# tobias-kirschstein/nersemble

Measured on NVIDIA H100. Metric: M ray-samples/sec, higher is better.
Workload: dtype f16 tables/MLP operands, f32 accumulate

## Files before the change

### nersemble_b200/csrc/nsb_field.cu

```cuda
#include <algorithm>
#include <cstdlib>
#include <cstring>

#define NSB_NO_SPIN_GUARD 1
#include "nsb_common.cuh"
#include "nsb_gather.cuh"
#include "nsb_march.cuh"
#include "nsb_mlp.cuh"
#include "nsb_tc.cuh"

namespace nsb {

constexpr int kSlabBytes = 2048;
constexpr int kChunkSlabs = 4;
constexpr int kChunkBytes = kSlabBytes * kChunkSlabs;
constexpr int kStages = 4;
constexpr int kBiasFloats = 6 * 128 + 8;

struct FieldArgs {
    nsb_field_params P;
    nsb_field_opts O;
    nsb_samples S;
    nsb_field_out out;
    float aabb_size[3];
// ... 198 lines not shown
        ha[0][1] = pack_h2(g02, b1acc[0][3]);
        ha[0][2] = pack_h2(b1acc[1][0], b1acc[1][1]);
        ha[0][3] = pack_h2(b1acc[1][2], b1acc[1][3]);
        float e[2][2];
#pragma unroll
        for (int h = 0; h < 2; ++h) {
            const int r = g + 8 * h;
            const float d0 = (dirsel[r][0] + 1.0f) / 2.0f, d1 = (dirsel[r][1] + 1.0f) / 2.0f,
                        d2 = (dirsel[r][2] + 1.0f) / 2.0f;
            e[h][0] = q == 0 ? d0 : (q == 1 ? d2 : 1.0f);
            e[h][1] = q == 0 ? d1 : 1.0f;
        }
        ha[1][0] = pack_h2(e[0][0], e[0][1]);
        ha[1][1] = pack_h2(e[1][0], e[1][1]);
        ha[1][2] = pack_h2(1.0f, 1.0f);
        ha[1][3] = pack_h2(1.0f, 1.0f);
    }
    float c0acc[8][4];
    smem_gemm<2, 4>(c0acc, ha, field_w + 384, lane);
    uint32_t c1in[4][4];
    relu_pack_nobias<8>(c0acc, c1in);
    float c1acc[8][4];
    smem_gemm<4, 4>(c1acc, c1in, field_w + 640, lane);
    uint32_t c2in[4][4];
    relu_pack_nobias<8>(c1acc, c2in);
    float c2acc[2][4];
    smem_gemm<4, 1>(c2acc, c2in, field_w + 1152, lane);
    if (A.out.rgb) {
        const int64_t sa = row0 + g, sb = row0 + g + 8;
        if (q == 0) {
            if (sa < n) { A.out.rgb[3 * sa + 0] = 1.f / (1.f + expf(-c2acc[0][0])); A.out.rgb[3 * sa + 1] = 1.f / (1.f + expf(-c2acc[0][1])); }
            if (sb < n) { A.out.rgb[3 * sb + 0] = 1.f / (1.f + expf(-c2acc[0][2])); A.out.rgb[3 * sb + 1] = 1.f / (1.f + expf(-c2acc[0][3])); }
        } else if (q == 1) {
            if (sa < n) A.out.rgb[3 * sa + 2] = 1.f / (1.f + expf(-c2acc[0][0]));
            if (sb < n) A.out.rgb[3 * sb + 2] = 1.f / (1.f + expf(-c2acc[0][2]));
        }
    }
}

template <bool DEFORM, bool FIELD, bool HEAD, bool SAVE>
__global__ void __launch_bounds__(kLaunchBoundWS, 1) field_kernel_ws(const __grid_constant__ FieldArgs A) {
    extern __shared__ __align__(1024) uint8_t smem_raw[];
    SmemWS &sm = *reinterpret_cast<SmemWS *>(smem_raw);
    const int tid = threadIdx.x, lane = tid & 31, warp = tid >> 5;
    constexpr bool FEAT_GIVEN = false;

#define NSB_N_SAMPLES A.S.n_samples
#include "nsb_field_setup.inc"
    if (warp >= kTensorWarps) {
        if (kGatherRegs != kLaunchRegs) asm volatile("setmaxnreg.dec.sync.aligned.u32 %0;" ::"n"(kGatherRegs));
#include "nsb_field_gather_role.inc"
        return;
    }

    if (kTensorRegs != kLaunchRegs) asm volatile("setmaxnreg.inc.sync.aligned.u32 %0;" ::"n"(kTensorRegs));
#include "nsb_field_tensor_role.inc"
#undef NSB_N_SAMPLES
}

template <bool DEFORM>
__global__ void __launch_bounds__(kLaunchBoundWS, 1) field_kernel_ws_given(const __grid_constant__ FieldArgs A) {
    extern __shared__ __align__(1024) uint8_t smem_raw[];
    SmemWS &sm = *reinterpret_cast<SmemWS *>(smem_raw);
    const int tid = threadIdx.x, lane = tid & 31, warp = tid >> 5;
    constexpr bool FIELD = true, HEAD = true, SAVE = true, FEAT_GIVEN = true;
#define NSB_N_SAMPLES A.S.n_samples
#include "nsb_field_setup.inc"
    if (warp >= kTensorWarps) {
        if (kGatherRegs != kLaunchRegs) asm volatile("setmaxnreg.dec.sync.aligned.u32 %0;" ::"n"(kGatherRegs));
#include "nsb_field_gather_role.inc"
        return;
    }
    if (kTensorRegs != kLaunchRegs) asm volatile("setmaxnreg.inc.sync.aligned.u32 %0;" ::"n"(kTensorRegs));
#include "nsb_field_tensor_role.inc"
#undef NSB_N_SAMPLES
}

#ifndef NSB_FRAME_GATHER_WARPS
#define NSB_FRAME_GATHER_WARPS 8
#endif
constexpr int kFrameGatherWarps = NSB_FRAME_GATHER_WARPS;
constexpr int kTcStages = 4, kTcBlocksPerTile = 14;
#ifdef NSB_TC_PROF
constexpr int kTcProfPhases = 9;
__device__ unsigned long long g_tc_prof[kTcProfPhases], g_tc_prof_k[8];
#define KPROF(i) if (threadIdx.x == 0 && blockIdx.x == 3) g_tc_prof_k[i] = (unsigned long long)clock64();
#else
#define KPROF(i)
#endif
constexpr size_t kTcPackedBytes = 12 * 16384 + 2 * 2048;

__device__ __forceinline__ int tc_warp_index(int tid) { return __shfl_sync(0xffffffffu, tid >> 5, 0); }

struct alignas(1024) SmemTC {
    uint8_t wring[kTcStages][16384];
    uint8_t a_enc[16384];
    uint4 field_w[kFieldPackedU4];
    alignas(16) float bias[kBiasFloats];
    alignas(16) float heads[2][64][8];
    uint64_t full[kTcStages];
    uint64_t xs_full[2], feat_full[2];
    uint32_t ring_rel[kTcStages];
    int row_ts[NSB_TILE];
    int tile_ctr[2];
    int64_t n_dyn;
    uint64_t sampler_done;
    alignas(16) float xs[2][NSB_TILE][4];
    alignas(16) __half feat[2][NSB_TILE * kFeatStride];
    alignas(16) float dirsel[2][NSB_TILE][4];
    uint2 blend_b[kGatherWarps][4 * 32];
    uint4 cv_stage[kGatherWarps][1];
};
static_assert(sizeof(SmemTC) <= 227 * 1024, "shared memory plan");
static_assert(kTensorWarps == 8, "the wgmma tensor role runs two warpgroups of 64 rows");

#define NSB_TC_SETUP()                                                                                              \
    {                                                                                                               \
        const uint4 *src = reinterpret_cast<const uint4 *>(A.P.field_packed);                                      \
        for (int i = tid; i < kFieldPackedU4; i += kThreadsWS) sm.field_w[i] = __ldg(src + i);                     \
        for (int i = tid; i < kBiasFloats; i += kThreadsWS) sm.bias[i] = __ldg(A.P.deform_bias + i);               \
        for (int i = tid; i < (int)(sizeof(sm.a_enc) / 16); i += kThreadsWS) reinterpret_cast<uint4 *>(&sm.a_enc)[i] = make_uint4(0u, 0u, 0u, 0u); \
        if (tid == 0) {                                                                                             \
            for (int s = 0; s < kTcStages; ++s) { mbar_init(&sm.full[s], 1); sm.ring_rel[s] = 0; }                \
            for (int b = 0; b < 2; ++b) {                                                                           \
                mbar_init(&sm.xs_full[b], kTensorWarps);                                                            \
                mbar_init(&sm.feat_full[b], kGatherWarps);                                                          \
                sm.tile_ctr[b] = 0;                                                                                 \
            }                                                                                                       \
            mbar_fence_init();                                                                                      \
        }                                                                                                           \
        __syncthreads();                                                                                            \
    }

template <bool HEAD, bool FRAME, bool STACK>
__global__ void __launch_bounds__(kLaunchBoundWS, 1) field_kernel_tc(const __grid_constant__ FieldArgs A) {
    extern __shared__ __align__(1024) uint8_t smem_raw[];
    SmemTC &sm = *reinterpret_cast<SmemTC *>(smem_raw);
    const int tid = threadIdx.x, lane = tid & 31, warp = tc_warp_index(tid);
    constexpr bool FIELD = true, SAVE = false, FEAT_GIVEN = false;
#define NSB_N_SAMPLES A.S.n_samples
    NSB_TC_SETUP()
    if (warp >= kTensorWarps) {
        if (kGatherRegs != kLaunchRegs) asm volatile("setmaxnreg.dec.sync.aligned.u32 %0;" ::"n"(kGatherRegs));
        if constexpr (FRAME) {
#include "nsb_field_gather_role_frame.inc"
        } else {
#include "nsb_field_gather_role.inc"
        }
        return;
    }
    if (kTensorRegs != kLaunchRegs) asm volatile("setmaxnreg.inc.sync.aligned.u32 %0;" ::"n"(kTensorRegs));
#include "nsb_field_tensor_role_tc.inc"
#undef NSB_N_SAMPLES
}

template <bool DEFORM, bool FIELD, bool HEAD, bool SAVE>
__global__ void __launch_bounds__(kLaunchBoundWS, 1) field_kernel_ws_dyn(const __grid_constant__ FieldArgs A) {
    extern __shared__ __align__(1024) uint8_t smem_raw[];
    SmemWS &sm = *reinterpret_cast<SmemWS *>(smem_raw);
    const int tid = threadIdx.x, lane = tid & 31, warp = tid >> 5;
    constexpr bool FEAT_GIVEN = false;
    if (tid == 0) sm.n_dyn = min(*A.S.n_samples_dev, A.S.n_samples);
#define NSB_N_SAMPLES (*reinterpret_cast<const volatile int64_t *>(&sm.n_dyn))
#include "nsb_field_setup.inc"
    if (warp >= kTensorWarps) {
        if (kGatherRegs != kLaunchRegs) asm volatile("setmaxnreg.dec.sync.aligned.u32 %0;" ::"n"(kGatherRegs));
#include "nsb_field_gather_role.inc"
        return;
    }
    if (kTensorRegs != kLaunchRegs) asm volatile("setmaxnreg.inc.sync.aligned.u32 %0;" ::"n"(kTensorRegs));
#include "nsb_field_tensor_role.inc"
#undef NSB_N_SAMPLES
}

struct RenderKArgs {
    FieldArgs F;
    nsb_march_args M;
    nsb_composite_args C;
    int32_t sampler, n_per_ray;
    float near_plane;
    int64_t capacity;
    nsb_render_ws_header *hdr;
    int64_t *partials;
    int64_t *packed_info;
};

__device__ __forceinline__ uint32_t ld_acquire_u32(const uint32_t *p) {
    uint32_t v;
    asm volatile("ld.acquire.gpu.global.u32 %0, [%1];" : "=r"(v) : "l"(p) : "memory");
    return v;
}
__device__ __forceinline__ void phase_sync() { asm volatile("bar.sync 1, %0;" ::"n"(kTensorWarps * 32) : "memory"); }
__device__ __forceinline__ void grid_barrier(uint32_t *ctr, const uint32_t target) {
    phase_sync();
    if (threadIdx.x == 0) {
        __threadfence();
        atomicAdd(ctr, 1u);
        while (ld_acquire_u32(ctr) < target) __nanosleep(40);
        __threadfence();
    }
    phase_sync();
}

__device__ __forceinline__ int64_t phase_sum_i64(int64_t v, int64_t *smem_warp , const int tid) {
// ... 208 lines not shown
    nsb_field_params P;
    nsb_field_opts O;
    const float *x;
    const float *codes;
    int64_t n;
    void *out;
    int out_is_half;
};

__global__ void __launch_bounds__(256) hash_blend_kernel(const __grid_constant__ HashArgs H) {
    const int lane = threadIdx.x & 31;
    const int64_t warp_global = (int64_t)blockIdx.x * (blockDim.x >> 5) + (threadIdx.x >> 5);
    const int64_t n_warps = (int64_t)gridDim.x * (blockDim.x >> 5);
    for (int64_t s = warp_global; s < H.n; s += n_warps) {
        const float x = H.x[3 * s + 0], y = H.x[3 * s + 1], z = H.x[3 * s + 2];
#if NSB_GATHER_MMA
        const BlendB Bf = make_blend_b(H.O, H.codes + s * NSB_MEMBERS, lane);
        const float val = gather_blend_mma(H.P, x, y, z, Bf, lane);
#else
        const int mg = lane & 7;
        float4 c = __ldg(reinterpret_cast<const float4 *>(H.codes + s * NSB_MEMBERS) + mg);
        float cw[4];
        cw[0] = fmaf(c.x, H.O.cw_scale[4 * mg + 0], H.O.cw_bias[4 * mg + 0]);
        cw[1] = fmaf(c.y, H.O.cw_scale[4 * mg + 1], H.O.cw_bias[4 * mg + 1]);
        cw[2] = fmaf(c.z, H.O.cw_scale[4 * mg + 2], H.O.cw_bias[4 * mg + 2]);
        cw[3] = fmaf(c.w, H.O.cw_scale[4 * mg + 3], H.O.cw_bias[4 * mg + 3]);
        const float val = gather_blend<2>(H.P, x, y, z, cw, lane);
#endif
        if (H.out_is_half)
            reinterpret_cast<__half *>(H.out)[s * 32 + lane] = __float2half_rn(val);
        else
            reinterpret_cast<float *>(H.out)[s * 32 + lane] = val;
    }
}

static int g_num_sms = 0;
static int num_sms() {
    if (g_num_sms == 0) {
        int dev = 0;
        cudaGetDevice(&dev);
        cudaDeviceGetAttribute(&g_num_sms, cudaDevAttrMultiProcessorCount, dev);
        if (g_num_sms <= 0) g_num_sms = 132;
    }
    return g_num_sms;
}

template <bool D, bool F, bool H, bool SV>
static int launch_field_ws_(const FieldArgs &A, cudaStream_t st) {
    const size_t smem = sizeof(SmemWS);
    static bool configured = false;
    if (!configured) {
        cudaError_t e = cudaFuncSetAttribute(field_kernel_ws<D, F, H, SV>, cudaFuncAttributeMaxDynamicSharedMemorySize, (int)smem);
        if (e != cudaSuccess) {
            set_error("cudaFuncSetAttribute(field_kernel_ws): %s", cudaGetErrorString(e));
            return 1;
        }
        configured = true;
    }
    const int64_t n_tiles = (A.S.n_samples + NSB_TILE - 1) / NSB_TILE;
    const int grid = (int)std::min<int64_t>(n_tiles, (int64_t)num_sms());
    field_kernel_ws<D, F, H, SV><<<grid, kThreadsWS, smem, st>>>(A);
    return check_launch("field_kernel_ws");
}
template <bool D, bool F, bool H, bool SV>
static int launch_field_ws_dyn_(const FieldArgs &A, cudaStream_t st) {
    const size_t smem = sizeof(SmemWS);
    static bool configured = false;
    if (!configured) {
        cudaError_t e = cudaFuncSetAttribute(field_kernel_ws_dyn<D, F, H, SV>, cudaFuncAttributeMaxDynamicSharedMemorySize, (int)smem);
        if (e != cudaSuccess) { set_error("cudaFuncSetAttribute(field_kernel_ws_dyn): %s", cudaGetErrorString(e)); return 1; }
        configured = true;
    }
    const int64_t n_tiles = (A.S.n_samples + NSB_TILE - 1) / NSB_TILE;
    const int grid = (int)std::min<int64_t>(n_tiles, (int64_t)num_sms());
    field_kernel_ws_dyn<D, F, H, SV><<<grid, kThreadsWS, smem, st>>>(A);
    return check_launch("field_kernel_ws_dyn");
}
template <bool D, bool F, bool H>
static int launch_field_ws(const FieldArgs &A, cudaStream_t st) {
    const bool save = A.out.xs || A.out.deform_acts || A.out.deform_enc || A.out.corner_vals;
    return save ? launch_field_ws_<D, F, H, true>(A, st) : launch_field_ws_<D, F, H, false>(A, st);
}

template <bool H, bool FR, bool ST>
static int launch_field_tc_(const FieldArgs &A, cudaStream_t st) {
    const size_t smem = sizeof(SmemTC);
    static bool configured = false;
    if (!configured) {
        cudaError_t e = cudaFuncSetAttribute(field_kernel_tc<H, FR, ST>, cudaFuncAttributeMaxDynamicSharedMemorySize, (int)smem);
        if (e != cudaSuccess) { set_error("cudaFuncSetAttribute(field_kernel_tc): %s", cudaGetErrorString(e)); return 1; }
        configured = true;
    }
    const int64_t n_tiles = (A.S.n_samples + NSB_TILE - 1) / NSB_TILE;
    const int grid = (int)std::min<int64_t>(n_tiles, (int64_t)num_sms());
    field_kernel_tc<H, FR, ST><<<grid, kThreadsWS, smem, st>>>(A);
    return check_launch("field_kernel_tc");
}
template <bool H>
static int launch_field_tc(const FieldArgs &A, cudaStream_t st) {
    if (!A.P.frame_table) return launch_field_tc_<H, false, false>(A, st);
    return A.P.frame_stride ? launch_field_tc_<H, true, true>(A, st) : launch_field_tc_<H, true, false>(A, st);
}

template <bool D>
static int launch_field_given(const FieldArgs &A, cudaStream_t st) {
    const size_t smem = sizeof(SmemWS);
    static bool configured = false;
    if (!configured) {
        cudaError_t e = cudaFuncSetAttribute(field_kernel_ws_given<D>, cudaFuncAttributeMaxDynamicSharedMemorySize, (int)smem);
        if (e != cudaSuccess) { set_error("cudaFuncSetAttribute(field_kernel_ws_given): %s", cudaGetErrorString(e)); return 1; }
        configured = true;
    }
    const int64_t n_tiles = (A.S.n_samples + NSB_TILE - 1) / NSB_TILE;
    const int grid = (int)std::min<int64_t>(n_tiles, (int64_t)num_sms());
    field_kernel_ws_given<D><<<grid, kThreadsWS, smem, st>>>(A);
    return check_launch("field_kernel_ws_given");
}

static bool frame_stride_ok(const nsb_field_params *p) {
    return p->frame_stride >= 0 && p->frame_stride * (int64_t)p->n_timesteps <= (int64_t)UINT32_MAX;
}

template <bool D, bool F, bool H>
static int launch_field(const FieldArgs &A, cudaStream_t st) {
    if (A.S.given_feat) {
        if (F && H && !A.S.n_samples_dev) return launch_field_given<D>(A, st);
        set_error("nsb_field_forward: given_feat needs the full evaluation (rgb) and a host-side sample count");
        return 1;
    }
    if (A.S.n_samples_dev) {
        if (F && !H) return launch_field_ws_dyn_<D, true, false, true>(A, st);
        set_error("nsb_field_forward: n_samples_dev is supported for the density evaluation (no rgb) only");
        return 1;
    }
    if (D && F && A.P.deform_packed_umma && !A.S.sample_code_bias && !(A.out.xs || A.out.deform_acts || A.out.deform_enc || A.out.corner_vals || A.out.feat))
        return launch_field_tc<H>(A, st);
    return launch_field_ws<D, F, H>(A, st);
}

}

using namespace nsb;

extern "C" size_t nsb_deform_packed_bytes(void) { return (size_t)kTbNumSlabs * kSlabBytes; }
extern "C" size_t nsb_field_packed_bytes(void) { return kFieldPackedU4 * sizeof(uint4); }
extern "C" size_t nsb_deform_packed_umma_bytes(void) { return kTcPackedBytes; }
#ifdef NSB_TC_PROF
extern "C" int nsb_debug_tc_prof(unsigned long long *out) {
    return (int)cudaMemcpyFromSymbol(out, nsb::g_tc_prof, sizeof(unsigned long long) * kTcProfPhases);
}
extern "C" int nsb_debug_tc_prof_kernel(unsigned long long *out8) {
    return (int)cudaMemcpyFromSymbol(out8, nsb::g_tc_prof_k, sizeof(unsigned long long) * 8);
}
#endif

extern "C" int nsb_field_forward(const nsb_field_params *params, const nsb_field_opts *opts, const nsb_samples *samples,
                                 const nsb_field_out *out, void *stream) {
    if (!params || !opts || !samples || !out) { set_error("nsb_field_forward: null argument"); return 1; }
    if (samples->n_samples <= 0) return 0;
    if (params->levels.n_levels != NSB_MAX_LEVELS) { set_error("nsb_field_forward: n_levels must be 16"); return 1; }
    if (!samples->origins && !samples->positions) { set_error("nsb_field_forward: no sample source"); return 1; }
    if (samples->origins && (!samples->directions || !samples->t_starts || !samples->t_ends || !samples->ray_indices)) {
        set_error("nsb_field_forward: ray-based samples need directions, t_starts, t_ends, ray_indices");
        return 1;
    }
    const bool deform = opts->use_deformation != 0;
    const bool need_field = out->sigma || out->rgb || out->feat || out->xs;
    const bool head = opts->compute_rgb != 0 && out->rgb != nullptr;
    if (!need_field && !(deform && out->offsets)) { set_error("nsb_field_forward: no outputs requested"); return 1; }
    if (need_field && (!params->tables || !params->field_packed)) { set_error("nsb_field_forward: tables/field_packed missing"); return 1; }
    if (need_field && !params->blend_codes && !samples->sample_blend_codes) { set_error("nsb_field_forward: no blend codes"); return 1; }
    if (deform && (!params->deform_packed_tb || !params->deform_bias || (!params->deform_code_bias && !samples->sample_code_bias))) {
// ... 8 lines not shown
    if (!frame_stride_ok(params)) { set_error("nsb_field_forward: frame_stride out of range"); return 1; }
    FieldArgs A;
    A.P = *params; A.O = *opts; A.S = *samples; A.out = *out;
    for (int k = 0; k < 3; ++k) A.aabb_size[k] = params->aabb[3 + k] - params->aabb[k];
    cudaStream_t st = (cudaStream_t)stream;
    if (deform) {
        if (!need_field) return launch_field<true, false, false>(A, st);
        return head ? launch_field<true, true, true>(A, st) : launch_field<true, true, false>(A, st);
    }
    return head ? launch_field<false, true, true>(A, st) : launch_field<false, true, false>(A, st);
}

extern "C" int nsb_hash_blend_forward(const nsb_field_params *params, const nsb_field_opts *opts, const float *x,
                                      const float *codes, int64_t n, void *out, int32_t out_is_half, void *stream) {
    if (!params || !opts || !x || !codes || !out) { set_error("nsb_hash_blend_forward: null argument"); return 1; }
    if (n <= 0) return 0;
    if (params->levels.n_levels != NSB_MAX_LEVELS) { set_error("nsb_hash_blend_forward: n_levels must be 16"); return 1; }
    HashArgs H;
    H.P = *params; H.O = *opts; H.x = x; H.codes = codes; H.n = n; H.out = out; H.out_is_half = out_is_half;
    const int64_t warps_needed = n;
    const int blocks = (int)std::min<int64_t>((warps_needed + 7) / 8, (int64_t)num_sms() * 8);
    hash_blend_kernel<<<blocks, 256, 0, (cudaStream_t)stream>>>(H);
    return check_launch("hash_blend_kernel");
}

namespace nsb {
constexpr int kBlendMaxTimesteps = 256;
__global__ void __launch_bounds__(256) blend_tables_kernel(const uint4 *__restrict__ tables, const float *__restrict__ code,
                                                           const __grid_constant__ nsb_field_opts O, float2 *__restrict__ out,
                                                           int n_ts, int64_t n_entries) {
    __shared__ float4 cw_s[kBlendMaxTimesteps][8];
    const int lane = threadIdx.x & 31, sub = lane & 7;
    for (int i = threadIdx.x; i < n_ts * 8; i += blockDim.x) {
        const int t = i >> 3, s = i & 7;
        float cw[4];
#pragma unroll
        for (int k = 0; k < 4; ++k) cw[k] = fmaf(__ldg(code + t * NSB_MEMBERS + 4 * s + k), O.cw_scale[4 * s + k], O.cw_bias[4 * s + k]);
        cw_s[t][s] = make_float4(cw[0], cw[1], cw[2], cw[3]);
    }
    __syncthreads();
    const int64_t stride = (int64_t)gridDim.x * (blockDim.x >> 3);
    for (int64_t e = (int64_t)blockIdx.x * (blockDim.x >> 3) + (threadIdx.x >> 3); e < ((n_entries + 3) & ~(int64_t)3); e += stride) {
        float2 f[4] = {};
        if (e < n_entries) {
            const uint4 v = __ldcs(tables + e * 8 + sub);
            f[0] = unpack_h2(v.x); f[1] = unpack_h2(v.y); f[2] = unpack_h2(v.z); f[3] = unpack_h2(v.w);
        }
        for (int t = 0; t < n_ts; ++t) {
            const float4 c4 = cw_s[t][sub];
            const float cw[4] = {c4.x, c4.y, c4.z, c4.w};
            float f0 = 0.f, f1 = 0.f;
#pragma unroll
            for (int i = 0; i < 4; ++i) { f0 = fmaf(cw[i], f[i].x, f0); f1 = fmaf(cw[i], f[i].y, f1); }
#pragma unroll
            for (int o = 1; o < 8; o <<= 1) { f0 += __shfl_xor_sync(0xffffffffu, f0, o); f1 += __shfl_xor_sync(0xffffffffu, f1, o); }
            if (sub == 0 && e < n_entries) out[(int64_t)t * n_entries + e] = make_float2(f0, f1);
        }
    }
}
}

extern "C" int nsb_blend_tables(const nsb_field_params *params, const nsb_field_opts *opts, int32_t first_timestep,
                                int32_t n_timesteps, int64_t n_entries, void *out, void *stream) {
    if (!params || !opts || !out || !params->tables || !params->blend_codes) { set_error("nsb_blend_tables: null argument"); return 1; }
    if (first_timestep < 0 || n_timesteps < 1 || n_timesteps > kBlendMaxTimesteps || first_timestep > params->n_timesteps - n_timesteps) {
        set_error("nsb_blend_tables: timesteps [%d, %d + %d) out of range (n_timesteps %d, at most %d per call)", first_timestep,
                  first_timestep, n_timesteps, params->n_timesteps, kBlendMaxTimesteps);
        return 1;
    }
    if (n_entries <= 0) return 0;
    const int blocks = (int)std::min<int64_t>((n_entries + 31) / 32, (int64_t)num_sms() * 8);
    blend_tables_kernel<<<blocks, 256, 0, (cudaStream_t)stream>>>(reinterpret_cast<const uint4 *>(params->tables),
                                                                  params->blend_codes + (size_t)first_timestep * NSB_MEMBERS, *opts,
                                                                  reinterpret_cast<float2 *>(out), n_timesteps, n_entries);
    return check_launch("blend_tables_kernel");
}

namespace nsb {
constexpr size_t kRenderHdrBytes = 64, kRenderPartials = 1024;
static_assert(sizeof(nsb_render_ws_header) == kRenderHdrBytes, "workspace header layout");

template <int SAMPLER, bool FR, bool ST>
static int launch_render_tc_(const RenderKArgs &K, cudaStream_t st) {
    const size_t smem = sizeof(SmemTC);
    static bool configured = false;
    if (!configured) {
        cudaError_t e = cudaFuncSetAttribute(render_kernel_tc<SAMPLER, FR, ST>, cudaFuncAttributeMaxDynamicSharedMemorySize, (int)smem);
        if (e != cudaSuccess) { set_error("cudaFuncSetAttribute(render_kernel_tc): %s", cudaGetErrorString(e)); return 1; }
        configured = true;
    }
    const int grid = num_sms();
    if ((size_t)grid > kRenderPartials) { set_error("nsb_render_forward: more SMs than scan partials"); return 1; }
    cudaError_t e = cudaMemsetAsync(&K.hdr->barrier, 0, sizeof(uint32_t), st);
    if (e != cudaSuccess) { set_error("nsb_render_forward: memset: %s", cudaGetErrorString(e)); return 2; }
    void *kargs[] = {const_cast<RenderKArgs *>(&K)};
    e = cudaLaunchCooperativeKernel(reinterpret_cast<const void *>(render_kernel_tc<SAMPLER, FR, ST>), dim3(grid), dim3(kThreadsWS), kargs, smem, st);
    if (e != cudaSuccess) { set_error("render_kernel_tc: %s", cudaGetErrorString(e)); return 2; }
    return check_launch("render_kernel_tc");
}
template <int SAMPLER>
static int launch_render_tc(const RenderKArgs &K, cudaStream_t st) {
    if (!K.F.P.frame_table) return launch_render_tc_<SAMPLER, false, false>(K, st);
    return K.F.P.frame_stride ? launch_render_tc_<SAMPLER, true, true>(K, st) : launch_render_tc_<SAMPLER, true, false>(K, st);
}

template <bool D, int SAMPLER>
static int launch_render(const RenderKArgs &K, cudaStream_t st) {
    if constexpr (D && SAMPLER != 1)
        if (K.F.P.deform_packed_umma)
            return SAMPLER == 0 ? launch_render_tc<4>(K, st) : launch_render_tc<2>(K, st);
    const size_t smem = sizeof(SmemWS);
    static bool configured = false;
    if (!configured) {
        cudaError_t e = cudaFuncSetAttribute(render_kernel_ws<D, SAMPLER>, cudaFuncAttributeMaxDynamicSharedMemorySize, (int)smem);
        if (e != cudaSuccess) { set_error("cudaFuncSetAttribute(render_kernel_ws): %s", cudaGetErrorString(e)); return 1; }
        configured = true;
    }
    const int grid = num_sms();
    if ((size_t)grid > kRenderPartials) { set_error("nsb_render_forward: more SMs than scan partials"); return 1; }
    cudaError_t e = cudaMemsetAsync(&K.hdr->barrier, 0, sizeof(uint32_t), st);
    if (e != cudaSuccess) { set_error("nsb_render_forward: memset: %s", cudaGetErrorString(e)); return 2; }
    void *kargs[] = {const_cast<RenderKArgs *>(&K)};
    e = cudaLaunchCooperativeKernel(reinterpret_cast<const void *>(render_kernel_ws<D, SAMPLER>), dim3(grid), dim3(kThreadsWS),
                                    kargs, smem, st);
    if (e != cudaSuccess) { set_error("render_kernel_ws: %s", cudaGetErrorString(e)); return 2; }
    return check_launch("render_kernel_ws");
}
}

extern "C" size_t nsb_render_workspace_bytes(int64_t n_rays) {
    return kRenderHdrBytes + kRenderPartials * sizeof(int64_t) + (size_t)std::max<int64_t>(n_rays, 1) * sizeof(int32_t) + 64;
}

extern "C" int nsb_render_forward(const nsb_field_params *params, const nsb_field_opts *opts, const nsb_render_args *ra, void *stream) {
    if (!params || !opts || !ra) { set_error("nsb_render_forward: null argument"); return 1; }
    if (ra->n_rays <= 0) return 0;
    if (params->levels.n_levels != NSB_MAX_LEVELS) { set_error("nsb_render_forward: n_levels must be 16"); return 1; }
    const bool deform = opts->use_deformation != 0;
    if (!ra->origins || !ra->directions || !ra->t_starts || !ra->t_ends || !ra->ray_indices || !ra->sigma || !ra->rgb ||
        !ra->packed_info || !ra->out_rgb || !ra->out_acc || !ra->out_depth || !ra->workspace || (deform && !ra->offsets)) {
        set_error("nsb_render_forward: null buffer");
        return 1;
    }
    if (!params->tables || !params->field_packed || !params->blend_codes) { set_error("nsb_render_forward: tables/field_packed/blend_codes missing"); return 1; }
    if (deform && (!params->deform_packed_tb || !params->deform_bias || !params->deform_code_bias)) {
        set_error("nsb_render_forward: deformation parameters missing");
        return 1;
    }
    if (params->n_timesteps < 1 || ra->capacity <= 0) { set_error("nsb_render_forward: n_timesteps < 1 or capacity <= 0"); return 1; }
    if (!frame_stride_ok(params)) { set_error("nsb_render_forward: frame_stride out of range"); return 1; }
    if (ra->sampler == 0) {
        if (ra->n_per_ray <= 0 || ra->capacity < ra->n_rays * (int64_t)ra->n_per_ray) { set_error("nsb_render_forward: capacity < n_rays * n_per_ray"); return 1; }
    } else if (ra->sampler == 1 || ra->sampler == 3) {
        if (!ra->near_planes || !ra->far_planes || !ra->binaries || !ra->aabbs) { set_error("nsb_render_forward: occupancy sampler arguments"); return 1; }
        if (ra->levels < 1 || ra->levels > 8 || (ra->sampler == 3 && ra->levels != 1)) {
            set_error("nsb_render_forward: levels must be in [1,8] (1 for the single-launch variant)");
            return 1;
        }
    } else { set_error("nsb_render_forward: unknown sampler"); return 1; }
    uint8_t *ws = reinterpret_cast<uint8_t *>(ra->workspace);
    RenderKArgs K;
    memset(&K, 0, sizeof(K));
    K.hdr = reinterpret_cast<nsb_render_ws_header *>(ws);
    K.partials = reinterpret_cast<int64_t *>(ws + kRenderHdrBytes);
    int32_t *counts = reinterpret_cast<int32_t *>(ws + kRenderHdrBytes + kRenderPartials * sizeof(int64_t));
    K.F.P = *params; K.F.O = *opts;
    K.F.O.compute_rgb = 1;
    for (int k = 0; k < 3; ++k) K.F.aabb_size[k] = params->aabb[3 + k] - params->aabb[k];
    K.F.S.n_samples = 0;
    K.F.S.origins = ra->origins; K.F.S.directions = ra->directions; K.F.S.ray_times = ra->ray_times;
// ... 23 lines not shown
```

### nersemble_b200/csrc/nsb_field_tensor_role_tc.inc

```
#ifdef NSB_TC_PROF
    long long prof_t = clock64(), prof[kTcProfPhases] = {};
#define PROF(i) { const long long c_ = clock64(); prof[i] += c_ - prof_t; prof_t = c_; }
#else
#define PROF(i)
#endif
    const int64_t n = NSB_N_SAMPLES;
    const int64_t n_tiles = (n + NSB_TILE - 1) / NSB_TILE;
    const int64_t my_tiles = blockIdx.x < n_tiles ? (n_tiles - blockIdx.x + gridDim.x - 1) / gridDim.x : 0;
    const int g = warp >> 2;
    const bool sin_half = (warp & 2) == 0;
    const int row = g * 64 + (warp & 1) * 32 + lane;
    const float amin0 = A.P.aabb[0], amin1 = A.P.aabb[1], amin2 = A.P.aabb[2];
    uint32_t blk = 0;
    const uint32_t blk_total = (uint32_t)(my_tiles * kTcBlocksPerTile);
    const uint8_t *const wsrc = reinterpret_cast<const uint8_t *>(A.P.deform_packed_umma);
    const uint32_t a_enc_s = smem_u32(sm.a_enc);
    const int frow = (warp & 3) * 16 + (lane >> 2), fcol = 2 * (lane & 3);
    auto wg_sync = [&]() { asm volatile("bar.sync %0, 128;" ::"r"(5 + g) : "memory"); };

    auto spin_wait = [&](uint64_t *bar, uint32_t parity) {
        uint32_t spins = 0;
        while (!mbar_try_wait(bar, parity))
            if (++spins > (1u << 26)) __trap();
    };
    auto refill = [&](uint32_t gb) {
        if (gb >= blk_total) return;
        const uint32_t s = gb % kTcStages, j = gb % kTcBlocksPerTile;
        const uint32_t bytes = j < 12 ? 16384u : 2048u;
        const uint32_t off = j < 12 ? j * 16384u : 12u * 16384u + (j - 12) * 2048u;
        mbar_expect_tx(&sm.full[s], bytes);
        bulk_g2s(sm.wring[s], wsrc + off, bytes, &sm.full[s]);
    };
    if (warp == 0) {
        if (tc::elect_one())
            for (uint32_t gb = 0; gb < kTcStages; ++gb) refill(gb);
        __syncwarp();
    }

    auto wait_blocks = [&](int nb) {
        for (int kb = 0; kb < nb; ++kb) spin_wait(&sm.full[(blk + kb) % kTcStages], ((blk + kb) / kTcStages) & 1);
    };
    auto release_blocks = [&](int nb) {
        if (tc::elect_one())
            for (int kb = 0; kb < nb; ++kb) {
                const uint32_t gb = blk + kb;
                uint32_t prev;
                asm volatile("atom.acq_rel.cta.shared::cta.add.u32 %0, [%1], 1;"
                             : "=r"(prev) : "r"(smem_u32(&sm.ring_rel[gb % kTcStages])) : "memory");
                if ((prev & 7) == 7) refill(gb + kTcStages);
            }
        __syncwarp();
        blk += nb;
    };
    auto b_desc = [&](int kb, int ks, int nh) {
        return tc::smem_desc(smem_u32(sm.wring[(blk + kb) % kTcStages]) + (uint32_t)(nh * 8 * 1024 + ks * 256), 128u, 1024u);
    };
    auto enc_desc = [&](int ks) { return tc::smem_desc(a_enc_s + (uint32_t)(g * 8 * 1024 + ks * 256), 128u, 1024u); };
    auto epilogue_piece = [&](const float (&d)[32], uint32_t (&a)[8][4], const int nh, const float *b0row, const float *b1row,
                              const float *sbias) {
#pragma unroll
        for (int j = 0; j < 8; ++j) {
            const int col = nh * 64 + j * 8 + fcol;
            float2 b0, b1;
            if (b0row) {
                b0 = __ldg(reinterpret_cast<const float2 *>(b0row + col));
                b1 = __ldg(reinterpret_cast<const float2 *>(b1row + col));
            } else {
                b0 = *reinterpret_cast<const float2 *>(sbias + col);
                b1 = b0;
            }
            a[4 * nh + j / 2][2 * (j & 1) + 0] = tc::cvt_relu_h2(d[4 * j + 0] + b0.x, d[4 * j + 1] + b0.y);
            a[4 * nh + j / 2][2 * (j & 1) + 1] = tc::cvt_relu_h2(d[4 * j + 2] + b1.x, d[4 * j + 3] + b1.y);
        }
    };

    struct RowIdx { int ri; float mid; };
    struct RowIn { float px, py, pz, ddx, ddy, ddz, tt; };
    const bool ray_based = A.S.origins != nullptr;
    auto load_idx = [&](int64_t it) -> RowIdx {
        RowIdx q{-1, 0.f};
        if (!ray_based || it >= my_tiles) return q;
        const int64_t s = (blockIdx.x + it * gridDim.x) * NSB_TILE + row;
        if (s < n) { q.ri = A.S.ray_indices[s]; q.mid = __fadd_rn(A.S.t_starts[s], A.S.t_ends[s]); }
        return q;
    };
    auto load_inputs = [&](int64_t it, const RowIdx q) -> RowIn {
        RowIn r{0.f, 0.f, 0.f, 0.f, 0.f, 0.f, 0.f};
        if (it >= my_tiles) return r;
        if (ray_based) {
            if (q.ri >= 0) {
                const int64_t ri = q.ri;
                r.ddx = A.S.directions[3 * ri + 0]; r.ddy = A.S.directions[3 * ri + 1]; r.ddz = A.S.directions[3 * ri + 2];
                r.px = A.S.origins[3 * ri + 0]; r.py = A.S.origins[3 * ri + 1]; r.pz = A.S.origins[3 * ri + 2];
                if (A.S.ray_times) r.tt = A.S.ray_times[ri];
            }
            return r;
        }
        const int64_t s = (blockIdx.x + it * gridDim.x) * NSB_TILE + row;
        if (s < n) {
            r.px = A.S.positions[3 * s + 0]; r.py = A.S.positions[3 * s + 1]; r.pz = A.S.positions[3 * s + 2];
            r.ddx = r.ddy = r.ddz = 1.0f;
            if (A.S.sample_directions) {
                r.ddx = A.S.sample_directions[3 * s + 0]; r.ddy = A.S.sample_directions[3 * s + 1];
                r.ddz = A.S.sample_directions[3 * s + 2];
            }
            if (A.S.sample_times) r.tt = A.S.sample_times[s];
        }
        return r;
    };

    auto deform_stage = [&](int64_t it, RowIn in, float mid, RowIn &next, RowIdx &idx1) {
        const int64_t tile = blockIdx.x + it * gridDim.x;
        const int b = (int)(it & 1);
        const int64_t s = tile * NSB_TILE + row;
        PROF(0)
        if constexpr (!FRAME) {
            const RowIdx q0 = load_idx(it);
            in = load_inputs(it, q0);
            mid = q0.mid;
        }
        const float ddx = in.ddx, ddy = in.ddy, ddz = in.ddz, tt = in.tt;
        float px = in.px, py = in.py, pz = in.pz;
        if (ray_based) {
            px = __fadd_rn(px, __fmul_rn(__fmul_rn(ddx, mid), 0.5f));
            py = __fadd_rn(py, __fmul_rn(__fmul_rn(ddy, mid), 0.5f));
            pz = __fadd_rn(pz, __fmul_rn(__fmul_rn(ddz, mid), 0.5f));
        }
        int tsi = __float2int_rn(__fmul_rn(tt, (float)(A.P.n_timesteps - 1)));
        tsi = min(max(tsi, 0), A.P.n_timesteps - 1);
        if (A.S.sample_code_bias) tsi = (int)min(s, n - 1);
        if (sin_half) { sm.dirsel[b][row][0] = ddx; sm.dirsel[b][row][1] = ddy; sm.dirsel[b][row][2] = ddz; }
        auto normalise = [&](float (&q)[3]) {
            q[0] = __fdiv_rn(__fsub_rn(px, amin0), A.aabb_size[0]);
            q[1] = __fdiv_rn(__fsub_rn(py, amin1), A.aabb_size[1]);
            q[2] = __fdiv_rn(__fsub_rn(pz, amin2), A.aabb_size[2]);
        };
        float p[3];
        normalise(p);
        if (sin_half) *reinterpret_cast<float4 *>(sm.xs[b][row]) = make_float4(px, py, pz, __int_as_float(tsi));
        PROF(1)
#ifndef NSB_TC_SKIP_D
        {
            uint8_t *dst_row = sm.a_enc + (row >> 3) * 1024 + (row & 7) * 16;
            auto put = [&](int col, float v) {
                *reinterpret_cast<__half *>(dst_row + (col >> 3) * 128 + (col & 7) * 2) = __float2half_rn(v);
            };
            const float a0 = 6.283185307179586f * p[0], a1 = 6.283185307179586f * p[1], a2 = 6.283185307179586f * p[2];
            const int c0 = sin_half ? 0 : 21;
#pragma unroll 1
            for (int j = 0; j < 7; ++j) {
                const float sc = (float)(1 << j), w = A.O.pe_window[j];
                const float g0 = a0 * sc, g1 = a1 * sc, g2 = a2 * sc;
                put(c0 + j, w * tc::sin_reduced(sin_half ? g0 : g0 + 1.5707963267948966f));
                put(c0 + 7 + j, w * tc::sin_reduced(sin_half ? g1 : g1 + 1.5707963267948966f));
                put(c0 + 14 + j, w * tc::sin_reduced(sin_half ? g2 : g2 + 1.5707963267948966f));
            }
            if (!sin_half) { put(42, 6.283185307179586f * p[0]); put(43, 6.283185307179586f * p[1]); put(44, 6.283185307179586f * p[2]); }
        }
        if (sin_half) sm.row_ts[row] = tsi;
        PROF(2)
        tc::fence_proxy_async();
        wg_sync();
        PROF(3)
        const float *const gcb = A.S.sample_code_bias ? A.S.sample_code_bias : A.P.deform_code_bias;
        uint32_t a[8][4] = {};
#pragma unroll 1
        for (int l = 0; l < 6; ++l) {
            const int nb = l == 0 ? 1 : (l == 4 ? 3 : 2);
            const bool code = l == 0 || l == 4;
            wait_blocks(nb);
            const float *b0row = nullptr, *b1row = nullptr;
            if (code) {
                b0row = gcb + (size_t)sm.row_ts[g * 64 + frow] * 256 + (l == 4 ? 128 : 0);
                b1row = gcb + (size_t)sm.row_ts[g * 64 + frow + 8] * 256 + (l == 4 ? 128 : 0);
            }
            uint32_t a_next[8][4];
#pragma unroll
            for (int nh = 0; nh < 2; ++nh) {
                float d[32];
                tc::wg_fence();
                if (l > 0) {
#pragma unroll
                    for (int k = 0; k < 8; ++k) tc::mma_m64n64k16_rs(d, a[k], b_desc(k >> 2, k & 3, nh), k > 0);
                }
                if (code) {
#pragma unroll
                    for (int ks = 0; ks < 3; ++ks) tc::mma_m64n64k16(d, enc_desc(ks), b_desc(nb - 1, ks, nh), l > 0 || ks > 0);
                }
                tc::wg_commit();
                tc::wg_wait<0>();
                if (nh == 1) release_blocks(nb);
                PROF(4)
                epilogue_piece(d, a_next, nh, b0row, b1row, sm.bias + l * 128);
                if (code) { PROF(8) } else { PROF(5) }
            }
#pragma unroll
            for (int k = 0; k < 8; ++k)
#pragma unroll
                for (int q = 0; q < 4; ++q) a[k][q] = a_next[k][q];
        }
        float *const heads = sm.heads[g][0];
        wait_blocks(2);
        {
            float d[8];
            tc::wg_fence();
#pragma unroll
            for (int k = 0; k < 8; ++k) tc::mma_m64n16k16_rs(d, a[k], b_desc(k >> 2, k & 3, 0), k > 0);
            tc::wg_commit();
            tc::wg_wait<0>();
            release_blocks(2);
            *reinterpret_cast<float2 *>(heads + frow * 8 + fcol) = make_float2(d[0], d[1]);
            *reinterpret_cast<float2 *>(heads + (frow + 8) * 8 + fcol) = make_float2(d[2], d[3]);
        }
        wg_sync();
        PROF(4)
        float h[8];
        *reinterpret_cast<float4 *>(h) = *reinterpret_cast<const float4 *>(heads + (row & 63) * 8);
        *reinterpret_cast<float4 *>(h + 4) = *reinterpret_cast<const float4 *>(heads + (row & 63) * 8 + 4);
#else
        float h[8] = {0.f, 0.f, 0.f, 0.f, 0.f, 0.f, 0.f, 0.f};
#endif
        if (sin_half) {
            const float4 q = *reinterpret_cast<const float4 *>(sm.xs[b][row]);
            px = q.x; py = q.y; pz = q.z; tsi = __float_as_int(q.w);
            normalise(p);
            const float v3[3] = {h[0] + sm.bias[6 * 128 + 0], h[1] + sm.bias[6 * 128 + 1], h[2] + sm.bias[6 * 128 + 2]};
            const float r3[3] = {h[3] + sm.bias[6 * 128 + 3], h[4] + sm.bias[6 * 128 + 4], h[5] + sm.bias[6 * 128 + 5]};
            float pw[3];
            se3_apply(p, r3, v3, pw);
            const float o0 = pw[0] - p[0], o1 = pw[1] - p[1], o2 = pw[2] - p[2];
            if (A.out.offsets && s < n) { A.out.offsets[3 * s + 0] = o0; A.out.offsets[3 * s + 1] = o1; A.out.offsets[3 * s + 2] = o2; }
            const float wx = px + o0, wy = py + o1, wz = pz + o2;
            if (FIELD) {
                const float x = __fdiv_rn(__fsub_rn(wx, amin0), A.aabb_size[0]);
                const float y = __fdiv_rn(__fsub_rn(wy, amin1), A.aabb_size[1]);
                const float z = __fdiv_rn(__fsub_rn(wz, amin2), A.aabb_size[2]);
                const bool sel = (x > 0.f) && (x < 1.f) && (y > 0.f) && (y < 1.f) && (z > 0.f) && (z < 1.f);
                *reinterpret_cast<float4 *>(sm.xs[b][row]) = make_float4(sel ? x : 0.f, sel ? y : 0.f, sel ? z : 0.f, __int_as_float(tsi));
                sm.dirsel[b][row][3] = sel ? 1.f : 0.f;
                if (tid == 0) sm.tile_ctr[b] = 0;
            }
        }
        if (FIELD) {
            __syncwarp();
            if (lane == 0) mbar_arrive(&sm.xs_full[b]);
        }
        if constexpr (FRAME) {
            next = load_inputs(it + 1, idx1);
            idx1 = load_idx(it + 2);
        }
        PROF(6)
    };

    RowIdx i0{-1, 0.f}, i1{-1, 0.f};
    RowIn cur{0.f, 0.f, 0.f, 0.f, 0.f, 0.f, 0.f}, nxt = cur;
    if constexpr (FRAME) { i0 = load_idx(0); i1 = load_idx(1); cur = load_inputs(0, i0); }
    float mid = i0.mid;
#pragma unroll 1
    for (int64_t it = -1; it < my_tiles; ++it) {
        if (it + 1 < my_tiles) {
            const float mid_next = i1.mid;
            deform_stage(it + 1, cur, mid, nxt, i1);
            cur = nxt; mid = mid_next;
        }
        if (FIELD && it >= 0) {
            const int64_t tile = blockIdx.x + it * gridDim.x;
            const int b = (int)(it & 1);
            mbar_wait<100>(&sm.feat_full[b], (uint32_t)(it >> 1) & 1);
            PROF(0)
#ifndef NSB_TC_SKIP_F
            field_mlp_tile<HEAD>(A, sm.field_w, &sm.feat[b][(warp * 16) * kFeatStride], &sm.dirsel[b][warp * 16],
                                 tile * NSB_TILE + warp * 16, n, lane);
#endif
            PROF(7)
        }
    }
#ifdef NSB_TC_PROF
    if (tid == 33 && blockIdx.x == 3)
        for (int i = 0; i < kTcProfPhases; ++i) g_tc_prof[i] = (unsigned long long)prof[i];
#endif
```

Baseline: 778.0.

## Stage per-timestep code bias in swizzled shared memory for TC deform MLP

Copies the per-timestep deformation code-bias table into a bank-swizzled shared-memory region at kernel setup when there are at most 32 timesteps and a frame table is used. The code layers' epilogues then read the bias from shared memory instead of issuing scattered global loads per row. To make room, the encoding buffer shrinks to three k-slices with a 768-byte stride, and the static bias array drops the layers that are never read in smem. It also rejects per-sample code bias for the TC kernels and sizes dynamic shared memory from the timestep count, which may affect occupancy and carveout.

```diff
diff --git a/nersemble_b200/csrc/nsb_field.cu b/nersemble_b200/csrc/nsb_field.cu
--- a/nersemble_b200/csrc/nsb_field.cu
+++ b/nersemble_b200/csrc/nsb_field.cu
@@ -304,7 +304,7 @@
 constexpr int kFrameGatherWarps = NSB_FRAME_GATHER_WARPS;
 constexpr int kTcStages = 4, kTcBlocksPerTile = 14;
 #ifdef NSB_TC_PROF
-constexpr int kTcProfPhases = 9;
+constexpr int kTcProfPhases = 10;
 __device__ unsigned long long g_tc_prof[kTcProfPhases], g_tc_prof_k[8];
 #define KPROF(i) if (threadIdx.x == 0 && blockIdx.x == 3) g_tc_prof_k[i] = (unsigned long long)clock64();
 #else
@@ -314,11 +314,14 @@
 
 __device__ __forceinline__ int tc_warp_index(int tid) { return __shfl_sync(0xffffffffu, tid >> 5, 0); }
 
+constexpr int kTcCodeBiasRows = 32;
+constexpr int kTcBiasFloats = 4 * 128 + 8;
+
 struct alignas(1024) SmemTC {
     uint8_t wring[kTcStages][16384];
-    uint8_t a_enc[16384];
+    uint8_t a_enc[12288];
     uint4 field_w[kFieldPackedU4];
-    alignas(16) float bias[kBiasFloats];
+    alignas(16) float bias[kTcBiasFloats];
     alignas(16) float heads[2][64][8];
     uint64_t full[kTcStages];
     uint64_t xs_full[2], feat_full[2];
@@ -333,15 +336,36 @@
     uint2 blend_b[kGatherWarps][4 * 32];
     uint4 cv_stage[kGatherWarps][1];
 };
-static_assert(sizeof(SmemTC) <= 227 * 1024, "shared memory plan");
+template <bool FRAME>
+__host__ __device__ constexpr size_t tc_code_bias_offset() {
+    return (FRAME ? offsetof(SmemTC, blend_b) + 127 : offsetof(SmemTC, cv_stage) + sizeof(SmemTC::cv_stage) + 127) / 128 * 128;
+}
+template <bool FRAME>
+__host__ __device__ constexpr size_t tc_smem_bytes(int staged_rows) { return tc_code_bias_offset<FRAME>() + (size_t)staged_rows * 1024; }
+static_assert(tc_code_bias_offset<true>() % 128 == 0 && tc_code_bias_offset<false>() % 128 == 0, "code-bias swizzle");
+static_assert(tc_smem_bytes<false>(kTcCodeBiasRows) <= 227 * 1024, "shared memory plan");
+static_assert(tc_smem_bytes<true>(kTcCodeBiasRows) + 1024 <= 164 * 1024, "frame-table kernels: 164 KB carveout step");
 static_assert(kTensorWarps == 8, "the wgmma tensor role runs two warpgroups of 64 rows");
+template <bool FRAME>
+__host__ __device__ __forceinline__ int tc_code_bias_rows(int n_timesteps) {
+    return FRAME && n_timesteps <= kTcCodeBiasRows ? n_timesteps : 0;
+}
 
 #define NSB_TC_SETUP()                                                                                              \
     {                                                                                                               \
         const uint4 *src = reinterpret_cast<const uint4 *>(A.P.field_packed);                                      \
         for (int i = tid; i < kFieldPackedU4; i += kThreadsWS) sm.field_w[i] = __ldg(src + i);                     \
-        for (int i = tid; i < kBiasFloats; i += kThreadsWS) sm.bias[i] = __ldg(A.P.deform_bias + i);               \
+        for (int i = tid; i < kTcBiasFloats; i += kThreadsWS)                                                      \
+            sm.bias[i] = __ldg(A.P.deform_bias + (i < 3 * 128 ? 128 + i : 256 + i));       \
         for (int i = tid; i < (int)(sizeof(sm.a_enc) / 16); i += kThreadsWS) reinterpret_cast<uint4 *>(&sm.a_enc)[i] = make_uint4(0u, 0u, 0u, 0u); \
+        {                                                                                                           \
+            float *const cb_s = reinterpret_cast<float *>(smem_raw + tc_code_bias_offset<FRAME>());                \
+            const float4 *cb_g = reinterpret_cast<const float4 *>(A.P.deform_code_bias);                           \
+            for (int i = tid; i < tc_code_bias_rows<FRAME>(A.P.n_timesteps) * 64; i += kThreadsWS) {                      \
+                const int t = i >> 6, c = (i >> 1) & 15;         \
+                *reinterpret_cast<float4 *>(cb_s + t * 256 + ((i >> 5) & 1) * 128 + (c ^ (t & 3)) * 8 + (i & 1) * 4) = __ldg(cb_g + i); \
+            }                                                                                                       \
+        }                                                                                                           \
         if (tid == 0) {                                                                                             \
             for (int s = 0; s < kTcStages; ++s) { mbar_init(&sm.full[s], 1); sm.ring_rel[s] = 0; }                \
             for (int b = 0; b < 2; ++b) {                                                                           \
@@ -716,12 +740,22 @@
     return save ? launch_field_ws_<D, F, H, true>(A, st) : launch_field_ws_<D, F, H, false>(A, st);
 }
 
+static bool tc_args_ok(const FieldArgs &A) {
+    if (A.S.sample_code_bias || !A.P.deform_code_bias) {
+        set_error("tc kernels: the code bias must come from the per-timestep table deform_code_bias");
+        return false;
+    }
+    return true;
+}
+
 template <bool H, bool FR, bool ST>
 static int launch_field_tc_(const FieldArgs &A, cudaStream_t st) {
-    const size_t smem = sizeof(SmemTC);
+    if (!tc_args_ok(A)) return 1;
+    const size_t smem = tc_smem_bytes<FR>(tc_code_bias_rows<FR>(A.P.n_timesteps));
     static bool configured = false;
     if (!configured) {
-        cudaError_t e = cudaFuncSetAttribute(field_kernel_tc<H, FR, ST>, cudaFuncAttributeMaxDynamicSharedMemorySize, (int)smem);
+        cudaError_t e = cudaFuncSetAttribute(field_kernel_tc<H, FR, ST>, cudaFuncAttributeMaxDynamicSharedMemorySize,
+                                             (int)tc_smem_bytes<FR>(tc_code_bias_rows<FR>(kTcCodeBiasRows)));
         if (e != cudaSuccess) { set_error("cudaFuncSetAttribute(field_kernel_tc): %s", cudaGetErrorString(e)); return 1; }
         configured = true;
     }
@@ -896,10 +930,12 @@
 
 template <int SAMPLER, bool FR, bool ST>
 static int launch_render_tc_(const RenderKArgs &K, cudaStream_t st) {
-    const size_t smem = sizeof(SmemTC);
+    if (!tc_args_ok(K.F)) return 1;
+    const size_t smem = tc_smem_bytes<FR>(tc_code_bias_rows<FR>(K.F.P.n_timesteps));
     static bool configured = false;
     if (!configured) {
-        cudaError_t e = cudaFuncSetAttribute(render_kernel_tc<SAMPLER, FR, ST>, cudaFuncAttributeMaxDynamicSharedMemorySize, (int)smem);
+        cudaError_t e = cudaFuncSetAttribute(render_kernel_tc<SAMPLER, FR, ST>, cudaFuncAttributeMaxDynamicSharedMemorySize,
+                                             (int)tc_smem_bytes<FR>(tc_code_bias_rows<FR>(kTcCodeBiasRows)));
         if (e != cudaSuccess) { set_error("cudaFuncSetAttribute(render_kernel_tc): %s", cudaGetErrorString(e)); return 1; }
         configured = true;
     }
diff --git a/nersemble_b200/csrc/nsb_field_tensor_role_tc.inc b/nersemble_b200/csrc/nsb_field_tensor_role_tc.inc
--- a/nersemble_b200/csrc/nsb_field_tensor_role_tc.inc
+++ b/nersemble_b200/csrc/nsb_field_tensor_role_tc.inc
@@ -55,9 +55,21 @@
     auto b_desc = [&](int kb, int ks, int nh) {
         return tc::smem_desc(smem_u32(sm.wring[(blk + kb) % kTcStages]) + (uint32_t)(nh * 8 * 1024 + ks * 256), 128u, 1024u);
     };
-    auto enc_desc = [&](int ks) { return tc::smem_desc(a_enc_s + (uint32_t)(g * 8 * 1024 + ks * 256), 128u, 1024u); };
-    auto epilogue_piece = [&](const float (&d)[32], uint32_t (&a)[8][4], const int nh, const float *b0row, const float *b1row,
-                              const float *sbias) {
+    auto enc_desc = [&](int ks) { return tc::smem_desc(a_enc_s + (uint32_t)(g * 8 * 768 + ks * 256), 128u, 768u); };
+    const bool cb_staged = tc_code_bias_rows<FRAME>(A.P.n_timesteps) > 0;
+    auto epilogue_piece = [&](const float (&d)[32], uint32_t (&a)[8][4], const int nh, const bool code, const uint32_t r0,
+                              const uint32_t r1, const float *b0row, const float *b1row, const float *sbias) {
+        if (code && cb_staged) {
+#pragma unroll
+            for (int j = 0; j < 8; ++j) {
+                const uint32_t o = (uint32_t)(nh * 2 + j / 4) * 128u, m = (uint32_t)(j & 3) << 5;
+                const float2 b0 = *reinterpret_cast<const float2 *>(smem_raw + (r0 ^ m) + o);
+                const float2 b1 = *reinterpret_cast<const float2 *>(smem_raw + (r1 ^ m) + o);
+                a[4 * nh + j / 2][2 * (j & 1) + 0] = tc::cvt_relu_h2(d[4 * j + 0] + b0.x, d[4 * j + 1] + b0.y);
+                a[4 * nh + j / 2][2 * (j & 1) + 1] = tc::cvt_relu_h2(d[4 * j + 2] + b1.x, d[4 * j + 3] + b1.y);
+            }
+            return;
+        }
 #pragma unroll
         for (int j = 0; j < 8; ++j) {
             const int col = nh * 64 + j * 8 + fcol;
@@ -141,7 +153,7 @@
         PROF(1)
 #ifndef NSB_TC_SKIP_D
         {
-            uint8_t *dst_row = sm.a_enc + (row >> 3) * 1024 + (row & 7) * 16;
+            uint8_t *dst_row = sm.a_enc + (row >> 3) * 768 + (row & 7) * 16;
             auto put = [&](int col, float v) {
                 *reinterpret_cast<__half *>(dst_row + (col >> 3) * 128 + (col & 7) * 2) = __float2half_rn(v);
             };
@@ -162,17 +174,26 @@
         tc::fence_proxy_async();
         wg_sync();
         PROF(3)
-        const float *const gcb = A.S.sample_code_bias ? A.S.sample_code_bias : A.P.deform_code_bias;
         uint32_t a[8][4] = {};
 #pragma unroll 1
         for (int l = 0; l < 6; ++l) {
             const int nb = l == 0 ? 1 : (l == 4 ? 3 : 2);
             const bool code = l == 0 || l == 4;
             wait_blocks(nb);
+            PROF(9)
+            uint32_t r0 = 0, r1 = 0;
             const float *b0row = nullptr, *b1row = nullptr;
             if (code) {
-                b0row = gcb + (size_t)sm.row_ts[g * 64 + frow] * 256 + (l == 4 ? 128 : 0);
-                b1row = gcb + (size_t)sm.row_ts[g * 64 + frow + 8] * 256 + (l == 4 ? 128 : 0);
+                const uint32_t t0 = (uint32_t)sm.row_ts[g * 64 + frow], t1 = (uint32_t)sm.row_ts[g * 64 + frow + 8];
+                if (cb_staged) {
+                    const uint32_t rb = (uint32_t)tc_code_bias_offset<FRAME>() + (l == 4 ? 512u : 0u) + (uint32_t)fcol * 4u;
+                    r0 = rb + t0 * 1024u + ((t0 & 3u) << 5);
+                    r1 = rb + t1 * 1024u + ((t1 & 3u) << 5);
+                } else {
+                    const float *const gcb = A.S.sample_code_bias ? A.S.sample_code_bias : A.P.deform_code_bias;
+                    b0row = gcb + (size_t)t0 * 256 + (l == 4 ? 128 : 0);
+                    b1row = gcb + (size_t)t1 * 256 + (l == 4 ? 128 : 0);
+                }
             }
             uint32_t a_next[8][4];
 #pragma unroll
@@ -191,7 +212,7 @@
                 tc::wg_wait<0>();
                 if (nh == 1) release_blocks(nb);
                 PROF(4)
-                epilogue_piece(d, a_next, nh, b0row, b1row, sm.bias + l * 128);
+                epilogue_piece(d, a_next, nh, code, r0, r1, b0row, b1row, sm.bias + (l == 5 ? 3 : l - 1) * 128);
                 if (code) { PROF(8) } else { PROF(5) }
             }
 #pragma unroll
@@ -201,6 +222,7 @@
         }
         float *const heads = sm.heads[g][0];
         wait_blocks(2);
+        PROF(9)
         {
             float d[8];
             tc::wg_fence();
@@ -224,8 +246,8 @@
             const float4 q = *reinterpret_cast<const float4 *>(sm.xs[b][row]);
             px = q.x; py = q.y; pz = q.z; tsi = __float_as_int(q.w);
             normalise(p);
-            const float v3[3] = {h[0] + sm.bias[6 * 128 + 0], h[1] + sm.bias[6 * 128 + 1], h[2] + sm.bias[6 * 128 + 2]};
-            const float r3[3] = {h[3] + sm.bias[6 * 128 + 3], h[4] + sm.bias[6 * 128 + 4], h[5] + sm.bias[6 * 128 + 5]};
+            const float v3[3] = {h[0] + sm.bias[4 * 128 + 0], h[1] + sm.bias[4 * 128 + 1], h[2] + sm.bias[4 * 128 + 2]};
+            const float r3[3] = {h[3] + sm.bias[4 * 128 + 3], h[4] + sm.bias[4 * 128 + 4], h[5] + sm.bias[4 * 128 + 5]};
             float pw[3];
             se3_apply(p, r3, v3, pw);
             const float o0 = pw[0] - p[0], o1 = pw[1] - p[1], o2 = pw[2] - p[2];
```

Result: faster. 849.5 (median of 6 runs) (+9.2%).
